# ur-whitelab/hoomd-tf

Hardware: AMD Instinct MI355X
Metric: MD steps/sec + achieved HBM GB/s, 131072 particles NN=128 (131k-particle box of the BASELINE metric) (higher is better)
Workload: dtype f32

## Files before the change

### hoomd_tf_amd/csrc/standin.hip

```cpp
#include <cstdlib>

#include "htf_common.h"
#include "box_math.h"
#include "htf_standin.h"
#include "standin_gate.h"
#include "key_sort.h"

namespace htf {

template <typename T>
__global__ __launch_bounds__(256) void nve_step_kernel(typename Vec4<T>::type *__restrict__ pos,
                                                       typename Vec4<T>::type *__restrict__ vel,
                                                       const typename Vec4<T>::type *__restrict__ force,
                                                       unsigned N, T dt, SBox<T> b) {
    unsigned i = blockIdx.x * blockDim.x + threadIdx.x;
    if (i >= N) return;
    auto p = pos[i];
    auto v = vel[i];
    nve_advance<T>(p, v, force[i], dt, b);
    pos[i] = p;
    vel[i] = v;
}

template <typename T>
__global__ __launch_bounds__(1024) void max_disp_kernel(const typename Vec4<T>::type *__restrict__ pos,
                                                        const typename Vec4<T>::type *__restrict__ ref, unsigned N,
                                                        SBox<T> b, float *__restrict__ out) {
    __shared__ float s_max[16];
    unsigned i = blockIdx.x * blockDim.x + threadIdx.x;
    float d2 = 0.f;
    if (i < N) {
        auto p = pos[i];
        auto r = ref[i];
        T dx = mimg<T>(p.x - r.x, b.L[0], b.Linv[0], b.periodic[0]);
        T dy = mimg<T>(p.y - r.y, b.L[1], b.Linv[1], b.periodic[1]);
        T dz = mimg<T>(p.z - r.z, b.L[2], b.Linv[2], b.periodic[2]);
        d2 = (float)(dx * dx + dy * dy + dz * dz);
        if (!(d2 == d2)) d2 = 0.f;
    }
    for (int m = 1; m < 64; m <<= 1) d2 = fmaxf(d2, __shfl_xor(d2, m));
    if ((threadIdx.x & 63) == 0) s_max[threadIdx.x >> 6] = d2;
    __syncthreads();
    if (threadIdx.x < 16) {
        d2 = s_max[threadIdx.x];
        for (int m = 1; m < 16; m <<= 1) d2 = fmaxf(d2, __shfl_xor(d2, m));
        if (threadIdx.x == 0 && __float_as_uint(d2) > *(volatile unsigned *)out)
            atomicMax((unsigned *)out, __float_as_uint(d2));
    }
}

template <typename T>
__global__ __launch_bounds__(1024) void check_disp_kernel(const typename Vec4<T>::type *__restrict__ pos,
                                                          const typename Vec4<T>::type *__restrict__ ref, unsigned N,
                                                          SBox<T> b, unsigned *__restrict__ work, float *__restrict__ out,
                                                          float *__restrict__ h_out, htfs_mirror mirror) {
    __shared__ float s_max[16];
    __shared__ unsigned s_last;
    unsigned i = blockIdx.x * blockDim.x + threadIdx.x;
    float d2 = 0.f;
    if (i < N) {
        auto p = pos[i];
        auto r = ref[i];
        T dx = mimg<T>(p.x - r.x, b.L[0], b.Linv[0], b.periodic[0]);
        T dy = mimg<T>(p.y - r.y, b.L[1], b.Linv[1], b.periodic[1]);
        T dz = mimg<T>(p.z - r.z, b.L[2], b.Linv[2], b.periodic[2]);
        d2 = (float)(dx * dx + dy * dy + dz * dz);
        if (!(d2 == d2)) d2 = 0.f;
    }
    for (int m = 1; m < 64; m <<= 1) d2 = fmaxf(d2, __shfl_xor(d2, m));
    if ((threadIdx.x & 63) == 0) s_max[threadIdx.x >> 6] = d2;
    if (threadIdx.x == 0) s_last = 0u;
    __syncthreads();
    if (threadIdx.x < 16) {
        d2 = s_max[threadIdx.x];
        for (int m = 1; m < 16; m <<= 1) d2 = fmaxf(d2, __shfl_xor(d2, m));
        if (threadIdx.x == 0) {
            if (__float_as_uint(d2) > *(volatile unsigned *)work) atomicMax(work, __float_as_uint(d2));
            __threadfence();
            if (atomicAdd(work + 1, 1u) == gridDim.x - 1u) s_last = 1u;
        }
    }
    __syncthreads();
    if (s_last == 0u) return;
    for (unsigned m = 0; m < mirror.n; ++m) {
        const unsigned *src = (const unsigned *)mirror.src[m];
        unsigned *dst = (unsigned *)mirror.dst[m];
        for (unsigned w = threadIdx.x; w < mirror.words[m]; w += blockDim.x) dst[w] = __builtin_nontemporal_load(src + w);
    }
    __threadfence_system();
    __syncthreads();
    if (threadIdx.x == 0) {
        const float worst = __uint_as_float(atomicExch(work, 0u));
        const unsigned cycle = __float_as_uint(out[1]) + 1u;
        out[0] = worst;
        out[1] = __uint_as_float(cycle);
        work[1] = 0u;
        if (h_out != nullptr) {
            h_out[0] = worst;
            __threadfence_system();
            *(volatile unsigned *)(h_out + 1) = cycle;
        }
    }
}

template <typename T>
__device__ __forceinline__ int cell_coord(T x, T lo, T Linv, int n) {
    int c = (int)floor((x - lo) * Linv * (T)n);
    return c < 0 ? 0 : (c >= n ? n - 1 : c);
}

template <typename T>
__global__ __launch_bounds__(256) void cell_index_kernel(const typename Vec4<T>::type *__restrict__ pos, unsigned Ntot,
                                                         SBox<T> b, int nx, int ny, int nz,
                                                         unsigned *__restrict__ cell_of, Gate gate) {
    if (gate.closed()) return;
    unsigned i = blockIdx.x * blockDim.x + threadIdx.x;
    if (i >= Ntot) return;
    auto p = pos[i];
    if (is_inert(p.x)) {
        cell_of[i] = kDeadCell;
        return;
    }
    int cx = cell_coord<T>(p.x, b.lo[0], b.Linv[0], nx);
    int cy = cell_coord<T>(p.y, b.lo[1], b.Linv[1], ny);
    int cz = cell_coord<T>(p.z, b.lo[2], b.Linv[2], nz);
    cell_of[i] = (unsigned)((cz * ny + cy) * nx + cx);
}

constexpr unsigned kTagSide = 1u << 31;
constexpr unsigned kRangeWrapShift = 28u, kRangeLenMask = (1u << kRangeWrapShift) - 1u;
struct RangesArgs {
    int nx, ny, nz, wx, wy, wz, px, py, pz;
    const unsigned *cell_start;
    uint4 *table;
    unsigned *max_neigh;
};
__device__ __forceinline__ void cell_ranges_body(const unsigned t, const RangesArgs &a) {
    const int nx = a.nx, ny = a.ny, nz = a.nz, wx = a.wx, wy = a.wy, wz = a.wz, px = a.px, py = a.py, pz = a.pz;
    const unsigned *__restrict__ cell_start = a.cell_start;
    uint4 *__restrict__ table = a.table;
    unsigned *__restrict__ max_neigh = a.max_neigh;
    const int nrow = (2 * wy + 1) * (2 * wz + 1);
    if (t == 0) *max_neigh = 0u;
    const unsigned ncell = (unsigned)(nx * ny * nz);
    if (t >= ncell * (unsigned)nrow) return;
    const int c = (int)(t / nrow), r = (int)(t % nrow);
    const int cx = c % nx, cy = (c / nx) % ny, cz = c / (nx * ny);
    const int dz = r / (2 * wy + 1) - wz, dy = r % (2 * wy + 1) - wy;
    int a0 = cx - wx, a1 = cx + wx, b0 = 0, b1 = -1;
    if (a0 < 0) {
        if (px) { b0 = nx + a0; b1 = nx - 1; }
        a0 = 0;
    } else if (a1 >= nx) {
// ... 234 lines not shown
            const unsigned i = my_tag & ~kTagSide;
            if (i < N) {
                n_neigh[i] = cnt < pitch ? cnt : pitch;
                head_list[i] = i * pitch;
                if (cnt > *(volatile unsigned *)max_neigh) atomicMax(max_neigh, cnt);
            }
        }
    }
}

}

using namespace htf;

extern "C" int htfs_nve_step(void *d_pos, void *d_vel, const void *d_force, int dtype, unsigned N, double dt,
                             const htf_box *box, htf_stream stream) {
    HTF_REQUIRE(d_pos && d_vel && d_force && box, "htfs_nve_step: null pointer");
    if (N == 0) return HTF_OK;
    unsigned grid = (N + 255) / 256;
    if (dtype == HTF_F32)
        hipLaunchKernelGGL((nve_step_kernel<float>), dim3(grid), dim3(256), 0, (hipStream_t)stream, (float4 *)d_pos, (float4 *)d_vel, (const float4 *)d_force, N, (float)dt, make_sbox<float>(box));
    else
        hipLaunchKernelGGL((nve_step_kernel<double>), dim3(grid), dim3(256), 0, (hipStream_t)stream, (double4 *)d_pos, (double4 *)d_vel, (const double4 *)d_force, N, dt, make_sbox<double>(box));
    return check_launch("nve_step_kernel");
}

extern "C" int htfs_max_displacement2(const void *d_pos, const void *d_ref, int dtype, unsigned N, const htf_box *box,
                                      float *d_out, htf_stream stream) {
    HTF_REQUIRE(d_pos && d_ref && box && d_out, "htfs_max_displacement2: null pointer");
    if (N == 0) return HTF_OK;
    unsigned grid = (N + 1023) / 1024;
    if (dtype == HTF_F32)
        hipLaunchKernelGGL((max_disp_kernel<float>), dim3(grid), dim3(1024), 0, (hipStream_t)stream, (const float4 *)d_pos, (const float4 *)d_ref, N, make_sbox<float>(box), d_out);
    else
        hipLaunchKernelGGL((max_disp_kernel<double>), dim3(grid), dim3(1024), 0, (hipStream_t)stream, (const double4 *)d_pos, (const double4 *)d_ref, N, make_sbox<double>(box), d_out);
    return check_launch("max_disp_kernel");
}

extern "C" int htfs_check_displacement2(const void *d_pos, const void *d_ref, int dtype, unsigned N, const htf_box *box,
                                        unsigned *d_work, float *d_out, float *h_out, const htfs_mirror *mirror, htf_stream stream) {
    using namespace htf;
    HTF_REQUIRE(d_pos && d_ref && box && d_work && d_out, "htfs_check_displacement2: null pointer");
    HTF_REQUIRE(N > 0, "htfs_check_displacement2: no rows");
    htfs_mirror mr = {};
    if (mirror != nullptr) {
        mr = *mirror;
        HTF_REQUIRE(mr.n <= HTFS_MIRROR_MAX, "htfs_check_displacement2: %u mirrors (at most %d)", mr.n, HTFS_MIRROR_MAX);
        for (unsigned m = 0; m < mr.n; ++m)
            HTF_REQUIRE(mr.src[m] && mr.dst[m] && ((uintptr_t)mr.src[m] & 3) == 0 && ((uintptr_t)mr.dst[m] & 3) == 0,
                        "htfs_check_displacement2: mirror %u: null or unaligned pointer", m);
    }
    unsigned grid = (N + 1023) / 1024;
    if (dtype == HTF_F32)
        hipLaunchKernelGGL((check_disp_kernel<float>), dim3(grid), dim3(1024), 0, (hipStream_t)stream, (const float4 *)d_pos, (const float4 *)d_ref, N, make_sbox<float>(box), d_work, d_out, h_out, mr);
    else
        hipLaunchKernelGGL((check_disp_kernel<double>), dim3(grid), dim3(1024), 0, (hipStream_t)stream, (const double4 *)d_pos, (const double4 *)d_ref, N, make_sbox<double>(box), d_work, d_out, h_out, mr);
    return check_launch("check_disp_kernel");
}

namespace htf {
struct Reimage {
    double L[3], c[3];
};
template <typename T>
__device__ __forceinline__ T reimage1(T x, double L, double c) {
    return L > 0.0 ? (T)((double)x - L * rint(((double)x - c) / L)) : x;
}

template <typename V>
__global__ __launch_bounds__(256) void bins_finish_kernel(RangesArgs ra, unsigned nb_ranges, V *__restrict__ dest, const V *__restrict__ src,
                                                          const int *__restrict__ order, unsigned n, int type_split, V *__restrict__ ref,
                                                          unsigned n_ref, unsigned *__restrict__ counter, Reimage im, Gate gate) {
    if (gate.closed()) return;
    if (blockIdx.x < nb_ranges) {
        cell_ranges_body(blockIdx.x * blockDim.x + threadIdx.x, ra);
        return;
    }
    const unsigned i = (blockIdx.x - nb_ranges) * blockDim.x + threadIdx.x;
    if (i == 0 && counter != nullptr) *counter += 1u;
    if (i >= n || i >= ra.cell_start[ra.nx * ra.ny * ra.nz]) return;
    const unsigned k = (unsigned)order[i];
    V p = src[k];
    if (ref != nullptr && k < n_ref) ref[k] = p;
    p.x = reimage1(p.x, im.L[0], im.c[0]);
    p.y = reimage1(p.y, im.L[1], im.c[1]);
    p.z = reimage1(p.z, im.L[2], im.c[2]);
    set_tag(p.w, k | ((type_split >= 0 && scalar_as_int(p.w) >= type_split) ? kTagSide : 0u));
    dest[i] = p;
}

template <typename T>
__global__ __launch_bounds__(256) void cell_index_count_kernel(const typename Vec4<T>::type *__restrict__ pos, unsigned Ntot, SBox<T> b,
                                                               int nx, int ny, int nz, unsigned *__restrict__ cell_of,
                                                               unsigned *__restrict__ count, Reimage im, Gate gate) {
    if (gate.closed()) return;
    unsigned i = blockIdx.x * blockDim.x + threadIdx.x;
    if (i >= Ntot) return;
    auto p = pos[i];
    if (is_inert(p.x)) {
        cell_of[i] = kDeadCell;
        return;
    }
    int cx = cell_coord<T>(reimage1(p.x, im.L[0], im.c[0]), b.lo[0], b.Linv[0], nx);
    int cy = cell_coord<T>(reimage1(p.y, im.L[1], im.c[1]), b.lo[1], b.Linv[1], ny);
    int cz = cell_coord<T>(reimage1(p.z, im.L[2], im.c[2]), b.lo[2], b.Linv[2], nz);
    const unsigned c = (unsigned)((cz * ny + cy) * nx + cx);
    cell_of[i] = c;
    atomicAdd(&count[c], 1u);
}

template <typename V, bool TAG>
__global__ void gather4_kernel(V *__restrict__ dest, const V *__restrict__ src, const int *__restrict__ order, unsigned n,
                               int type_split, Gate gate, const unsigned *__restrict__ n_live = nullptr) {
    if (gate.closed()) return;
    const unsigned i = blockIdx.x * blockDim.x + threadIdx.x;
    if (i >= n) return;
    if (n_live != nullptr && i >= *n_live) return;
    const unsigned k = (unsigned)order[i];
    V p = src[k];
    if (TAG) set_tag(p.w, k | ((type_split >= 0 && scalar_as_int(p.w) >= type_split) ? kTagSide : 0u));
    dest[i] = p;
}
}

namespace htf {
__global__ __launch_bounds__(256) void cell_count_kernel(const unsigned *__restrict__ cell_of, unsigned n,
                                                         unsigned *__restrict__ count, Gate gate) {
    if (gate.closed()) return;
    const unsigned i = blockIdx.x * blockDim.x + threadIdx.x;
    if (i < n && cell_of[i] != kDeadCell) atomicAdd(&count[cell_of[i]], 1u);
}

constexpr unsigned kScanThreads = 256, kScanPer = 8, kScanChunk = kScanThreads * kScanPer;
__global__ __launch_bounds__(kScanThreads) void cell_scan_kernel(const unsigned *__restrict__ count, unsigned ncell,
                                                         unsigned *__restrict__ start, unsigned *__restrict__ cursor, Gate gate) {
    if (gate.closed()) return;
    __shared__ unsigned s_wave[kScanThreads / 64], s_carry[kScanThreads / 64];
    const unsigned t = threadIdx.x, lane = t & 63u, wave = t >> 6;
    const unsigned base = blockIdx.x * kScanChunk;
    unsigned before_blk = 0;
    {
// ... 18 lines not shown
        const unsigned v = (unsigned)__shfl_up((int)incl, off);
        if (lane >= off) incl += v;
    }
    if (lane == 63) s_wave[wave] = incl;
    __syncthreads();
    unsigned before = 0, total = 0, carry = 0;
#pragma unroll
    for (unsigned w = 0; w < kScanThreads / 64; ++w) {
        const unsigned v = s_wave[w];
        before += w < wave ? v : 0u;
        total += v;
        carry += s_carry[w];
    }
    unsigned run = carry + before + (incl - sum);
#pragma unroll
    for (unsigned i = 0; i < kScanPer; ++i)
        if (first + i < ncell) {
            start[first + i] = run;
            cursor[first + i] = run;
            run += c[i];
        }
    if (blockIdx.x == gridDim.x - 1 && t == 0) start[ncell] = carry + total;
}

__global__ __launch_bounds__(256) void cell_scatter_kernel(const unsigned *__restrict__ cell_of, unsigned n,
                                                           unsigned *__restrict__ cursor, unsigned *__restrict__ order, Gate gate) {
    if (gate.closed()) return;
    const unsigned i = blockIdx.x * blockDim.x + threadIdx.x;
    if (i < n && cell_of[i] != kDeadCell) order[atomicAdd(&cursor[cell_of[i]], 1u)] = i;
}

__global__ __launch_bounds__(256) void cell_order_kernel(const unsigned *__restrict__ start, unsigned ncell,
                                                         unsigned *__restrict__ order, unsigned *__restrict__ count, Gate gate) {
    if (gate.closed()) return;
    const unsigned c = blockIdx.x * blockDim.x + threadIdx.x;
    if (c >= ncell) return;
    count[c] = 0u;
    const unsigned b = start[c], e = start[c + 1];
    for (unsigned i = b + 1; i < e; ++i) {
        const unsigned v = order[i];
        unsigned j = i;
        while (j > b && order[j - 1] > v) {
            order[j] = order[j - 1];
            --j;
        }
        order[j] = v;
    }
}
}

static int zero_counts(unsigned *count, unsigned ncell, hipStream_t s) {
    HTF_REQUIRE(((uintptr_t)count & 15) == 0, "binning scratch must be 16-byte aligned (cell_scan_kernel reads it with 16-byte loads)");
    HTF_CHECK_HIP(hipMemsetAsync(count, 0, (size_t)ncell * sizeof(unsigned), s));
    return HTF_OK;
}

extern "C" int htfs_cell_sort(const unsigned *d_cell_of, unsigned Ntot, unsigned ncell, unsigned *d_scratch,
                              unsigned *d_cell_start, unsigned *d_order, htf_stream stream) {
    using namespace htf;
    HTF_REQUIRE(d_cell_of && d_scratch && d_cell_start && d_order, "htfs_cell_sort: null pointer");
    HTF_REQUIRE(ncell > 0, "htfs_cell_sort: no cells");
    hipStream_t s = (hipStream_t)stream;
    unsigned *count = d_scratch, *cursor = d_scratch + ncell;
    if (int rc = zero_counts(count, ncell, s)) return rc;
    if (Ntot) hipLaunchKernelGGL(cell_count_kernel, dim3((Ntot + 255) / 256), dim3(256), 0, s, d_cell_of, Ntot, count, kOpenGate);
    hipLaunchKernelGGL(cell_scan_kernel, dim3((ncell + kScanChunk - 1) / kScanChunk), dim3(kScanThreads), 0, s, count, ncell, d_cell_start, cursor, kOpenGate);
    if (Ntot) hipLaunchKernelGGL(cell_scatter_kernel, dim3((Ntot + 255) / 256), dim3(256), 0, s, d_cell_of, Ntot, cursor, d_order, kOpenGate);
    hipLaunchKernelGGL(cell_order_kernel, dim3((ncell + 255) / 256), dim3(256), 0, s, d_cell_start, ncell, d_order, count, kOpenGate);
    return check_launch("htfs_cell_sort");
}

static int gather4(void *d_dest, const void *d_src, const int *d_order, int dtype, unsigned n, bool tag, int type_split,
                   htf_stream stream, const unsigned *d_n_live = nullptr) {
    using namespace htf;
    HTF_REQUIRE(d_dest && d_src && d_order, "htfs_gather4_tagged: null pointer");
    HTF_REQUIRE(!tag || n <= kTagSide, "htfs_gather4_tagged: %u particles do not fit the 31-bit tag", n);
    if (n == 0) return HTF_OK;
    const dim3 grid((n + 255) / 256), block(256);
    hipStream_t s = (hipStream_t)stream;
    if (dtype == HTF_F32) {
        if (tag) hipLaunchKernelGGL((gather4_kernel<float4, true>), grid, block, 0, s, (float4 *)d_dest, (const float4 *)d_src, d_order, n, type_split, kOpenGate, d_n_live);
        else hipLaunchKernelGGL((gather4_kernel<float4, false>), grid, block, 0, s, (float4 *)d_dest, (const float4 *)d_src, d_order, n, type_split, kOpenGate, d_n_live);
    } else {
        if (tag) hipLaunchKernelGGL((gather4_kernel<double4, true>), grid, block, 0, s, (double4 *)d_dest, (const double4 *)d_src, d_order, n, type_split, kOpenGate, d_n_live);
        else hipLaunchKernelGGL((gather4_kernel<double4, false>), grid, block, 0, s, (double4 *)d_dest, (const double4 *)d_src, d_order, n, type_split, kOpenGate, d_n_live);
    }
    return check_launch("gather4_kernel");
}

extern "C" int htfs_gather4_tagged(void *d_dest, const void *d_src, const int *d_order, int dtype, unsigned n, int type_split,
                                   htf_stream stream) {
    return gather4(d_dest, d_src, d_order, dtype, n, true, type_split, stream);
}

extern "C" int htfs_gather4_tagged_live(void *d_dest, const void *d_src, const int *d_order, int dtype, unsigned n_max,
                                        const unsigned *d_n_live, int type_split, htf_stream stream) {
    HTF_REQUIRE(d_n_live, "htfs_gather4_tagged_live: null pointer");
    return gather4(d_dest, d_src, d_order, dtype, n_max, true, type_split, stream, d_n_live);
}

template <typename T, typename V4>
__global__ __launch_bounds__(256) void slab_classify_kernel(const V4 *__restrict__ pos, unsigned N, const T *__restrict__ bounds,
                                                            int world, int rank, T r_ghost, unsigned *__restrict__ key) {
    const unsigned i = blockIdx.x * blockDim.x + threadIdx.x;
    if (i >= N) return;
    const T x = pos[i].x;
// ... 40 lines not shown
                                                           unsigned row_words, SegTable t, unsigned total_rows) {
    const unsigned w = blockIdx.x * blockDim.x + threadIdx.x;
    if (w >= total_rows * row_words) return;
    unsigned row = w / row_words;
    const unsigned col = w - row * row_words;
    unsigned seg = 0;
#pragma unroll 1
    while (seg + 1 < t.n && row >= t.cnt[seg]) {
        row -= t.cnt[seg];
        ++seg;
    }
    dst[(size_t)(t.dst[seg] + row) * row_words + col] = src[(size_t)(t.src[seg] + row) * row_words + col];
}

extern "C" int htfs_segment_copy(void *d_dst, const void *d_src, unsigned row_bytes, unsigned n_segments,
                                 const unsigned *src_start, const unsigned *dst_start, const unsigned *count, htf_stream stream) {
    HTF_REQUIRE(d_dst && d_src && src_start && dst_start && count, "htfs_segment_copy: null pointer");
    HTF_REQUIRE(n_segments >= 1 && n_segments <= HTFS_MAX_SEGMENTS && row_bytes % 4 == 0 && row_bytes > 0,
                "htfs_segment_copy: need 1..%d segments of whole 32-bit words", HTFS_MAX_SEGMENTS);
    SegTable t;
    t.n = 0;
    unsigned total = 0;
    for (unsigned s = 0; s < n_segments; ++s) {
        if (count[s] == 0) continue;
        t.src[t.n] = src_start[s];
        t.dst[t.n] = dst_start[s];
        t.cnt[t.n] = count[s];
        total += count[s];
        ++t.n;
    }
    if (total == 0) return HTF_OK;
    const unsigned words = row_bytes / 4;
    const unsigned grid = (unsigned)(((size_t)total * words + 255) / 256);
    hipLaunchKernelGGL(segment_copy_kernel, dim3(grid), dim3(256), 0, (hipStream_t)stream, (unsigned *)d_dst, (const unsigned *)d_src,
                       words, t, total);
    return check_launch("segment_copy_kernel");
}

extern "C" int htfs_cell_index(const void *d_pos, int dtype, unsigned Ntot, const htf_box *box, const int *ncell3,
                               unsigned *d_cell_of, htf_stream stream) {
    HTF_REQUIRE(d_pos && box && ncell3 && d_cell_of, "htfs_cell_index: null pointer");
    if (Ntot == 0) return HTF_OK;
    unsigned grid = (Ntot + 255) / 256;
    if (dtype == HTF_F32)
        hipLaunchKernelGGL((cell_index_kernel<float>), dim3(grid), dim3(256), 0, (hipStream_t)stream, (const float4 *)d_pos, Ntot, make_sbox<float>(box), ncell3[0], ncell3[1], ncell3[2], d_cell_of, kOpenGate);
    else
        hipLaunchKernelGGL((cell_index_kernel<double>), dim3(grid), dim3(256), 0, (hipStream_t)stream, (const double4 *)d_pos, Ntot, make_sbox<double>(box), ncell3[0], ncell3[1], ncell3[2], d_cell_of, kOpenGate);
    return check_launch("cell_index_kernel");
}

struct FinishArgs {
    unsigned n;
    htf::Reimage im;
};

static int build_nlist_impl(const htfs_nlist *l, const void *d_pos, int dtype, unsigned N, htf_stream stream, htf::Gate gate,
                            const FinishArgs *fin) {
    using namespace htf;
    HTF_REQUIRE(l && d_pos && l->pos_sorted && l->cell_start && l->n_neigh && l->head_list && l->nlist && l->max_neigh,
                "htfs_build_nlist: null pointer");
    const htf_box *box = &l->box;
    const int *ncell3 = l->ncell3, *stencil3 = l->stencil3;
    const unsigned *d_cell_start = l->cell_start;
    const void *d_pos_sorted = l->pos_sorted;
    const unsigned pitch = l->pitch;
    const int type_split = l->type_split;
    const double r_list = l->r_list;
    unsigned *d_n_neigh = l->n_neigh, *d_head_list = l->head_list, *d_nlist = l->nlist, *d_max_neigh = l->max_neigh;
    HTF_REQUIRE(pitch > 0, "htfs_build_nlist: pitch must be > 0");
    for (int d = 0; d < 3; ++d) {
        const double w = (box->hi[d] - box->lo[d]) / ncell3[d];
        const int sw = stencil3[d];
        HTF_REQUIRE((sw == 0 && ncell3[d] == 1) || (sw >= 1 && sw <= 2 && ncell3[d] >= 2 * sw + 1 && w * sw >= r_list * (1.0 - 1e-12)),
                    "htfs_build_nlist: along %d need 1 cell, or >= 2w+1 cells with w cells spanning r_list (got %d cells of %g, stencil %d, r_list %g)",
                    d, ncell3[d], w, sw, r_list);
    }
    if (N == 0) return HTF_OK;
    const unsigned ncell = (unsigned)(ncell3[0] * ncell3[1] * ncell3[2]);
    const unsigned nrow = (unsigned)((2 * stencil3[1] + 1) * (2 * stencil3[2] + 1));
    HTF_REQUIRE(l->ranges && ((uintptr_t)l->ranges & 15) == 0, "htfs_build_nlist: ranges must be a 16-byte aligned table of 4 * ncell * rows words");
    uint4 *d_ranges = (uint4 *)l->ranges;
    const RangesArgs ra = {ncell3[0], ncell3[1], ncell3[2], stencil3[0], stencil3[1], stencil3[2], (int)box->periodic[0],
                           (int)box->periodic[1], (int)box->periodic[2], d_cell_start, d_ranges, d_max_neigh};
    const unsigned nb_ranges = (ncell * nrow + 255) / 256;
    if (fin == nullptr) {
        hipLaunchKernelGGL(cell_ranges_kernel, dim3(nb_ranges), dim3(256), 0, (hipStream_t)stream, ra, gate);
    } else {
        const unsigned nb = nb_ranges + (fin->n + 255) / 256 + (fin->n == 0 ? 1u : 0u);
        if (dtype == HTF_F32)
            hipLaunchKernelGGL((bins_finish_kernel<float4>), dim3(nb), dim3(256), 0, (hipStream_t)stream, ra, nb_ranges, (float4 *)l->pos_sorted,
                               (const float4 *)d_pos, (const int *)l->order, fin->n, type_split, (float4 *)l->ref, N, l->counter, fin->im, gate);
        else
            hipLaunchKernelGGL((bins_finish_kernel<double4>), dim3(nb), dim3(256), 0, (hipStream_t)stream, ra, nb_ranges, (double4 *)l->pos_sorted,
                               (const double4 *)d_pos, (const int *)l->order, fin->n, type_split, (double4 *)l->ref, N, l->counter, fin->im, gate);
    }
    const bool fine = stencil3[0] == 2 || stencil3[1] == 2 || stencil3[2] == 2;
#define HTFS_NL(T, V4, G)                                                                                              \
    if (shift) HTFS_NL_(T, V4, G, true); else HTFS_NL_(T, V4, G, false)
#define HTFS_NL_(T, V4, G, S)                                                                                          \
    hipLaunchKernelGGL((build_nlist_kernel<T, G, S>), dim3((N + 4 * (64 / G) - 1) / (4 * (64 / G))), dim3(256), 0, (hipStream_t)stream, \
                       (const V4 *)d_pos, (const V4 *)d_pos_sorted, N, make_sbox<T>(box), (T)(r_list * r_list), ncell3[0],  \
                       ncell3[1], ncell3[2], stencil3[0], stencil3[1], stencil3[2], d_cell_start, pitch,      \
                       type_split, d_n_neigh, d_head_list, d_nlist, d_max_neigh, (const uint4 *)d_ranges, gate)
#define HTFS_NLC(T, V4)                                                                                                \
    if (shift) HTFS_NLC_(T, V4, true); else HTFS_NLC_(T, V4, false)
#define HTFS_NLC_(T, V4, S)                                                                                            \
    hipLaunchKernelGGL((build_nlist_cells_kernel<T, S>), dim3((ncell * cell_split + 3) / 4), dim3(256), 0, (hipStream_t)stream, \
                       (const V4 *)d_pos_sorted, N, make_sbox<T>(box), (T)(r_list * r_list), ncell, (int)nrow, d_cell_start, pitch, \
                       type_split, d_n_neigh, d_head_list, d_nlist, d_max_neigh, (const uint4 *)d_ranges, cell_split, gate)
    bool shift = true;
    for (int d = 0; d < 3; ++d) shift = shift && (!box->periodic[d] || ncell3[d] >= 7);
#ifdef HTF_AB_VARIANTS
    static const bool per_particle = std::getenv("HTFS_NLIST_PER_PARTICLE") != nullptr, per_cell = std::getenv("HTFS_NLIST_PER_CELL") != nullptr;
#else
    constexpr bool per_particle = false, per_cell = false;
#endif
    const bool reimaged = fin != nullptr && (fin->im.L[0] > 0.0 || fin->im.L[1] > 0.0 || fin->im.L[2] > 0.0);
    const bool by_cell = per_cell || reimaged || (!per_particle && ncell >= 1024u);
    const unsigned cell_split = ncell <= 12288u ? 2u : 1u;
    if (by_cell) {
        if (dtype == HTF_F32) { HTFS_NLC(float, float4); } else { HTFS_NLC(double, double4); }
    } else if (dtype == HTF_F32) {
        if (fine) { HTFS_NL(float, float4, 8); } else { HTFS_NL(float, float4, 16); }
    } else {
        if (fine) { HTFS_NL(double, double4, 8); } else { HTFS_NL(double, double4, 16); }
    }
#undef HTFS_NL
#undef HTFS_NL_
#undef HTFS_NLC
#undef HTFS_NLC_
    return check_launch("build_nlist_kernel");
}

extern "C" int htfs_build_nlist(const htfs_nlist *nl, const void *d_pos, int dtype, unsigned N, htf_stream stream) {
    return build_nlist_impl(nl, d_pos, dtype, N, stream, htf::kOpenGate, nullptr);
}

static int rebuild_nlist_impl(const htfs_nlist *l, const void *d_pos, int dtype, unsigned N, unsigned Ntot, bool scratch_clean,
                              htf_stream stream, htf::Gate gate) {
    using namespace htf;
    HTF_REQUIRE(l && d_pos && l->cell_of && l->scratch && l->cell_start && l->order && l->pos_sorted, "htfs_rebuild_nlist: null pointer");
    HTF_REQUIRE(Ntot >= N, "htfs_rebuild_nlist: Ntot %u < N %u", Ntot, N);
    if (N == 0) return HTF_OK;
    const htf_box *box = &l->box;
    const int *ncell3 = l->ncell3;
    const unsigned ncell = (unsigned)(ncell3[0] * ncell3[1] * ncell3[2]);
    HTF_REQUIRE(ncell > 0, "htfs_rebuild_nlist: no cells");
    hipStream_t s = (hipStream_t)stream;
    unsigned *count = l->scratch, *cursor = l->scratch + ncell;
    if (!scratch_clean)
        if (int rc = zero_counts(count, ncell, s)) return rc;
    const unsigned grid = (Ntot + 255) / 256;
    Reimage im = {};
    for (int d = 0; d < 3; ++d) {
        im.L[d] = !box->periodic[d] ? l->image_L[d] : 0.0;
        im.c[d] = 0.5 * (box->lo[d] + box->hi[d]);
        HTF_REQUIRE(im.L[d] == 0.0 || im.L[d] >= box->hi[d] - box->lo[d], "htfs_rebuild_nlist: image length %g along axis %d is shorter than the grid", im.L[d], d);
    }
    if (dtype == HTF_F32)
        hipLaunchKernelGGL((cell_index_count_kernel<float>), dim3(grid), dim3(256), 0, s, (const float4 *)d_pos, Ntot, make_sbox<float>(box),
                           ncell3[0], ncell3[1], ncell3[2], l->cell_of, count, im, gate);
    else
        hipLaunchKernelGGL((cell_index_count_kernel<double>), dim3(grid), dim3(256), 0, s, (const double4 *)d_pos, Ntot, make_sbox<double>(box),
                           ncell3[0], ncell3[1], ncell3[2], l->cell_of, count, im, gate);
    hipLaunchKernelGGL(cell_scan_kernel, dim3((ncell + kScanChunk - 1) / kScanChunk), dim3(kScanThreads), 0, s, count, ncell, l->cell_start, cursor, gate);
    hipLaunchKernelGGL(cell_scatter_kernel, dim3(grid), dim3(256), 0, s, l->cell_of, Ntot, cursor, l->order, gate);
    hipLaunchKernelGGL(cell_order_kernel, dim3((ncell + 255) / 256), dim3(256), 0, s, l->cell_start, ncell, l->order, count, gate);
    const FinishArgs fin = {Ntot, im};
    return build_nlist_impl(l, d_pos, dtype, N, stream, gate, &fin);
}

extern "C" int htfs_rebuild_nlist(const htfs_nlist *nl, const void *d_pos, int dtype, unsigned N, unsigned Ntot, int scratch_clean,
                                  htf_stream stream) {
    return rebuild_nlist_impl(nl, d_pos, dtype, N, Ntot, scratch_clean != 0, stream, htf::kOpenGate);
}

extern "C" int htfs_check_rebuild_nlist(const htfs_nlist *nl, const void *d_pos, int dtype, unsigned N, unsigned Ntot, int scratch_clean,
                                        float *d_disp2, double threshold2, unsigned *d_stat2, unsigned *h_stat2, htf_stream stream) {
    HTF_REQUIRE(nl && nl->ref && d_disp2 && d_stat2, "htfs_check_rebuild_nlist: null pointer");
    if (N == 0) return HTF_OK;
    HTF_CHECK_HIP(hipMemsetAsync(d_disp2, 0, sizeof(float), (hipStream_t)stream));
    int rc = htfs_max_displacement2(d_pos, nl->ref, dtype, N, &nl->box, d_disp2, stream);
    if (rc != HTF_OK) return rc;
    htfs_nlist l = *nl;
    l.max_neigh = d_stat2;
    l.counter = d_stat2 + 1;
    rc = rebuild_nlist_impl(&l, d_pos, dtype, N, Ntot, scratch_clean != 0, stream, htf::Gate{d_disp2, (float)threshold2});
    if (rc != HTF_OK) return rc;
    if (h_stat2 != nullptr)
        HTF_CHECK_HIP(hipMemcpyAsync(h_stat2, d_stat2, 2 * sizeof(unsigned), hipMemcpyDeviceToHost, (hipStream_t)stream));
    return HTF_OK;
}
```

### hoomd_tf_amd/standin.py

```python
import ctypes as C
import math
import os

import numpy as np
import torch

from . import _lib, ops
from ._lib import lib, check
from .ops import raw_stream


def fcc_positions(n_cells, rho):
    a = (4.0 / rho) ** (1.0 / 3.0)
    L = n_cells * a
    ijk = np.stack(np.meshgrid(*[np.arange(n_cells)] * 3, indexing="ij"), -1).reshape(-1, 3)
    base = np.array([[0.25, 0.25, 0.25], [0.75, 0.75, 0.25], [0.75, 0.25, 0.75], [0.25, 0.75, 0.75]])
    pos = ((ijk[:, None, :] + base[None]) * a).reshape(-1, 3) - L / 2
    return pos, np.array([L, L, L]), a


def sc_positions(n_cells, rho):
    a = (1.0 / rho) ** (1.0 / 3.0)
    L = n_cells * a
    ijk = np.stack(np.meshgrid(*[np.arange(n_cells)] * 3, indexing="ij"), -1).reshape(-1, 3)
# ... 123 lines not shown
        self._capturing = False
        self._stat = self._stat_host = self._stat_event = None
        self._max_host = self._max_event = None
        self._mirrored = False

    def subscribe(self, rcut_fn):
        self._subscribers.append(rcut_fn)
        self.r_cut = max([self.r_cut] + [float(fn()) for fn in self._subscribers])
        self._ref = None

    @property
    def r_list(self):
        return self.r_cut + self.r_buff

    def _ncell(self):
        b3, _ = self._search_box()
        L = b3[1] - b3[0]
        n = np.ones(3, dtype=int)
        w = np.zeros(3, dtype=int)
        for d in range(3):
            fine = int(np.floor(L[d] / (self.r_list / 2.0)))
            coarse = int(np.floor(L[d] / self.r_list))
            if fine >= 5:
                n[d], w[d] = fine, 2
            elif coarse >= 3:
                n[d], w[d] = coarse, 1
        return n, w

    def _search_box(self):
        if self.domain is not None and getattr(self.domain, "local_grid", False):
            return self.domain.nlist_box()
        return self.sys.box3x3, self.sys.periodic

    def _size_grid(self):
        s, d = self.sys, self._desc
        b3, per = self._search_box()
        key = (np.asarray(b3).tobytes(), per)
        if self._sbox_key != key:
            self._sbox_key = key
            d.box = _lib.make_box(np.asarray(b3), per)
        n, w = self._ncell()
        ncell = int(n[0] * n[1] * n[2])
        Ntot = s.N + s.n_ghost
        d.r_list = self.r_list
        d.ncell3[:] = [int(x) for x in n]
        d.stencil3[:] = [int(x) for x in w]
        lengths = getattr(self.domain, "image_lengths", None)
        d.image_L[:] = lengths() if lengths is not None else (0.0, 0.0, 0.0)
        if self._scr_n != (Ntot, ncell, int(w[1]), int(w[2])):
            self._scr_n = (Ntot, ncell, int(w[1]), int(w[2]))
            self._cell_of = torch.empty(Ntot, dtype=torch.int32, device=s.device)
            self._order = torch.empty(Ntot, dtype=torch.int32, device=s.device)
            self._cell_start = torch.empty(ncell + 1, dtype=torch.int32, device=s.device)
            self._bin_scratch = torch.empty(2 * ncell, dtype=torch.int32, device=s.device)
            self._pos_sorted = torch.empty((Ntot, 4), dtype=s.pos.dtype, device=s.device)
            self._ranges = torch.empty(4 * ncell * int((2 * w[1] + 1) * (2 * w[2] + 1)), dtype=torch.int32, device=s.device)
            d.cell_of, d.order, d.cell_start = self._cell_of.data_ptr(), self._order.data_ptr(), self._cell_start.data_ptr()
            d.scratch, d.pos_sorted, d.ranges = self._bin_scratch.data_ptr(), self._pos_sorted.data_ptr(), self._ranges.data_ptr()
        self._grid = (n, w, ncell)
        return Ntot

    def build(self):
        s = self.sys
        if self.domain is not None:
            self.domain.rebuild()
        Ntot = self._size_grid()
        fixed = self.domain is not None and getattr(self.domain, "fixed_capacity", False)
        if (fixed and self.n_builds > 0 and not self.sort_particles and self._ref is not None and self._ref.shape[0] == s.N
                and self.nlist is not None and self.nlist.numel() == s.N * self.pitch):
            self._rebuild_fixed(Ntot)
        else:
            self._build_sized(Ntot, fixed)
        if self._rule is not None:
            self._rule.reset()
            self._dd_prev = None
        self.n_builds += 1

    def _rebuild_fixed(self, Ntot):
        self._poll_max()
        self._enqueue_rebuild(Ntot, gated=False)
        self._copy_max_late()

    def _build_sized(self, Ntot, fixed):
        s, d = self.sys, self._desc
        n, _, ncell = self._grid
        cell_of = self._cell_of
        stream = C.c_void_p(raw_stream(s.device.index))
        check(lib.htfs_cell_index(s.pos.data_ptr(), s.scalar_code, Ntot, C.byref(d.box), C.byref(d.ncell3), d.cell_of, stream))
        if self.sort_particles and s.N > 0:
            key = cell_of[: s.N].to(torch.int64)
            if self.domain is not None and self.domain.world > 1:
                key = key + self.domain.row_classes() * ncell
            perm = torch.sort(key, stable=True)[1]
            s.pos[: s.N] = s.pos[: s.N].index_select(0, perm)
            s.vel = s.vel.index_select(0, perm)
            cell_of[: s.N] = cell_of[: s.N].index_select(0, perm)
        self._scratch_clean = None
        check(lib.htfs_cell_sort(d.cell_of, Ntot, ncell, d.scratch, d.cell_start, d.order, stream))
        self._scratch_clean = (d.scratch, ncell)
        if fixed:
            check(lib.htfs_gather4_tagged_live(d.pos_sorted, s.pos.data_ptr(), d.order, s.scalar_code, Ntot,
                                               d.cell_start + 4 * ncell, int(self.type_split), stream))
        else:
            check(lib.htfs_gather4_tagged(d.pos_sorted, s.pos.data_ptr(), d.order, s.scalar_code, Ntot, int(self.type_split), stream))
        if self.pitch is None:
            L = s.box3x3[1] - s.box3x3[0]
            n_real = getattr(self.domain, "n_global", None) if fixed else None
# ... 656 lines not shown
```

### include/htf_standin.h

```cpp
#ifndef HTF_STANDIN_H_
#define HTF_STANDIN_H_
#include "htf_amd.h"
#ifdef __cplusplus
extern "C" {
#endif

HTF_API int htfs_nve_step(void *d_pos, void *d_vel, const void *d_force, int dtype, unsigned N,
                          double dt, const htf_box *box, htf_stream stream);

HTF_API int htfs_max_displacement2(const void *d_pos, const void *d_ref, int dtype, unsigned N,
                                   const htf_box *box, float *d_out, htf_stream stream);

#define HTFS_MIRROR_MAX 4
typedef struct htfs_mirror {
    const void *src[HTFS_MIRROR_MAX];
    void *dst[HTFS_MIRROR_MAX];
    unsigned words[HTFS_MIRROR_MAX];
    unsigned n;
} htfs_mirror;
HTF_API int htfs_check_displacement2(const void *d_pos, const void *d_ref, int dtype, unsigned N, const htf_box *box,
                                     unsigned *d_work, float *d_out, float *h_out, const htfs_mirror *mirror, htf_stream stream);

#define HTFS_RANGE_WORDS(ncell, stencil_y, stencil_z) (4u * (size_t)(ncell) * (2u * (stencil_y) + 1u) * (2u * (stencil_z) + 1u))
typedef struct htfs_nlist {
    htf_box box;
    double r_list;
    int ncell3[3];
    int stencil3[3];
    unsigned pitch;
    int type_split;
    unsigned *cell_of;
    unsigned *scratch;
    unsigned *cell_start;
    unsigned *order;
    void *pos_sorted;
    void *ranges;
    unsigned *n_neigh;
    unsigned *head_list;
    unsigned *nlist;
    unsigned *max_neigh;
    void *ref;
    unsigned *counter;
    double image_L[3];
} htfs_nlist;

HTF_API int htfs_cell_index(const void *d_pos, int dtype, unsigned Ntot, const htf_box *box,
                            const int *ncell3, unsigned *d_cell_of, htf_stream stream);
HTF_API int htfs_cell_sort(const unsigned *d_cell_of, unsigned Ntot, unsigned ncell, unsigned *d_scratch,
                           unsigned *d_cell_start, unsigned *d_order, htf_stream stream);
HTF_API int htfs_gather4_tagged(void *d_dest, const void *d_src, const int *d_order, int dtype, unsigned n, int type_split,
                                htf_stream stream);
HTF_API int htfs_gather4_tagged_live(void *d_dest, const void *d_src, const int *d_order, int dtype, unsigned n_max,
                                     const unsigned *d_n_live, int type_split, htf_stream stream);
HTF_API int htfs_build_nlist(const htfs_nlist *nl, const void *d_pos, int dtype, unsigned N, htf_stream stream);

HTF_API int htfs_rebuild_nlist(const htfs_nlist *nl, const void *d_pos, int dtype, unsigned N, unsigned Ntot, int scratch_clean,
                               htf_stream stream);

HTF_API int htfs_check_rebuild_nlist(const htfs_nlist *nl, const void *d_pos, int dtype, unsigned N, unsigned Ntot, int scratch_clean,
                                     float *d_disp2, double threshold2, unsigned *d_stat2, unsigned *h_stat2, htf_stream stream);

HTF_API int htfs_slab_classify(const void *d_pos, int dtype, unsigned N, const void *d_bounds, int world, int rank,
                               double r_ghost, unsigned *d_key, htf_stream stream);

HTF_API int htfs_key_sort16(const unsigned *d_key, unsigned N, unsigned *d_scratch, unsigned *d_start, unsigned *d_order,
                            htf_stream stream);

#define HTFS_MAX_SEGMENTS 16
HTF_API int htfs_segment_copy(void *d_dst, const void *d_src, unsigned row_bytes, unsigned n_segments,
                              const unsigned *src_start, const unsigned *dst_start, const unsigned *count, htf_stream stream);

#define HTFS_BRICK_MAX_MSG 8
#define HTFS_BRICK_MAX_P 64
typedef struct htfs_brick {
    int ndim;
    int axis[2];
// ... 123 lines not shown
```

Measured before the change: 13280.

## Fold cell ordering into bins_finish and fuse displacement check with counter reset

Removes the separate cell_order_kernel. The scatter now writes into a staging buffer, and bins_finish computes each particle's deterministic in-cell slot by counting smaller indices within its cell, while also zeroing the cell counts. The nlist rebuild check replaces a memset plus max_disp launch with a single check_disp_kernel variant that resets its work counters itself, so later memsets are skipped. The cost is an O(cell occupancy) scan per particle and a larger scratch buffer.

```diff
diff --git a/hoomd_tf_amd/csrc/standin.hip b/hoomd_tf_amd/csrc/standin.hip
--- a/hoomd_tf_amd/csrc/standin.hip
+++ b/hoomd_tf_amd/csrc/standin.hip
@@ -23,10 +23,9 @@
 }
 
 template <typename T>
-__global__ __launch_bounds__(1024) void max_disp_kernel(const typename Vec4<T>::type *__restrict__ pos,
-                                                        const typename Vec4<T>::type *__restrict__ ref, unsigned N,
-                                                        SBox<T> b, float *__restrict__ out) {
-    __shared__ float s_max[16];
+__device__ __forceinline__ float block_max_disp2(const typename Vec4<T>::type *__restrict__ pos,
+                                                 const typename Vec4<T>::type *__restrict__ ref, unsigned N, const SBox<T> &b,
+                                                 float *s_max) {
     unsigned i = blockIdx.x * blockDim.x + threadIdx.x;
     float d2 = 0.f;
     if (i < N) {
@@ -44,61 +43,57 @@
     if (threadIdx.x < 16) {
         d2 = s_max[threadIdx.x];
         for (int m = 1; m < 16; m <<= 1) d2 = fmaxf(d2, __shfl_xor(d2, m));
-        if (threadIdx.x == 0 && __float_as_uint(d2) > *(volatile unsigned *)out)
-            atomicMax((unsigned *)out, __float_as_uint(d2));
-    }
+    }
+    return d2;
 }
 
 template <typename T>
+__global__ __launch_bounds__(1024) void max_disp_kernel(const typename Vec4<T>::type *__restrict__ pos,
+                                                        const typename Vec4<T>::type *__restrict__ ref, unsigned N,
+                                                        SBox<T> b, float *__restrict__ out) {
+    __shared__ float s_max[16];
+    const float d2 = block_max_disp2<T>(pos, ref, N, b, s_max);
+    if (threadIdx.x == 0 && __float_as_uint(d2) > *(volatile unsigned *)out)
+        atomicMax((unsigned *)out, __float_as_uint(d2));
+}
+
+template <typename T, bool CYCLE>
 __global__ __launch_bounds__(1024) void check_disp_kernel(const typename Vec4<T>::type *__restrict__ pos,
                                                           const typename Vec4<T>::type *__restrict__ ref, unsigned N,
                                                           SBox<T> b, unsigned *__restrict__ work, float *__restrict__ out,
                                                           float *__restrict__ h_out, htfs_mirror mirror) {
     __shared__ float s_max[16];
     __shared__ unsigned s_last;
-    unsigned i = blockIdx.x * blockDim.x + threadIdx.x;
-    float d2 = 0.f;
-    if (i < N) {
-        auto p = pos[i];
-        auto r = ref[i];
-        T dx = mimg<T>(p.x - r.x, b.L[0], b.Linv[0], b.periodic[0]);
-        T dy = mimg<T>(p.y - r.y, b.L[1], b.Linv[1], b.periodic[1]);
-        T dz = mimg<T>(p.z - r.z, b.L[2], b.Linv[2], b.periodic[2]);
-        d2 = (float)(dx * dx + dy * dy + dz * dz);
-        if (!(d2 == d2)) d2 = 0.f;
-    }
-    for (int m = 1; m < 64; m <<= 1) d2 = fmaxf(d2, __shfl_xor(d2, m));
-    if ((threadIdx.x & 63) == 0) s_max[threadIdx.x >> 6] = d2;
     if (threadIdx.x == 0) s_last = 0u;
-    __syncthreads();
-    if (threadIdx.x < 16) {
-        d2 = s_max[threadIdx.x];
-        for (int m = 1; m < 16; m <<= 1) d2 = fmaxf(d2, __shfl_xor(d2, m));
-        if (threadIdx.x == 0) {
-            if (__float_as_uint(d2) > *(volatile unsigned *)work) atomicMax(work, __float_as_uint(d2));
-            __threadfence();
-            if (atomicAdd(work + 1, 1u) == gridDim.x - 1u) s_last = 1u;
-        }
+    const float d2 = block_max_disp2<T>(pos, ref, N, b, s_max);
+    if (threadIdx.x == 0) {
+        if (__float_as_uint(d2) > *(volatile unsigned *)work) atomicMax(work, __float_as_uint(d2));
+        __threadfence();
+        if (atomicAdd(work + 1, 1u) == gridDim.x - 1u) s_last = 1u;
     }
     __syncthreads();
     if (s_last == 0u) return;
-    for (unsigned m = 0; m < mirror.n; ++m) {
-        const unsigned *src = (const unsigned *)mirror.src[m];
-        unsigned *dst = (unsigned *)mirror.dst[m];
-        for (unsigned w = threadIdx.x; w < mirror.words[m]; w += blockDim.x) dst[w] = __builtin_nontemporal_load(src + w);
-    }
-    __threadfence_system();
-    __syncthreads();
+    if (CYCLE) {
+        for (unsigned m = 0; m < mirror.n; ++m) {
+            const unsigned *src = (const unsigned *)mirror.src[m];
+            unsigned *dst = (unsigned *)mirror.dst[m];
+            for (unsigned w = threadIdx.x; w < mirror.words[m]; w += blockDim.x) dst[w] = __builtin_nontemporal_load(src + w);
+        }
+        __threadfence_system();
+        __syncthreads();
+    }
     if (threadIdx.x == 0) {
         const float worst = __uint_as_float(atomicExch(work, 0u));
-        const unsigned cycle = __float_as_uint(out[1]) + 1u;
         out[0] = worst;
-        out[1] = __uint_as_float(cycle);
         work[1] = 0u;
-        if (h_out != nullptr) {
-            h_out[0] = worst;
-            __threadfence_system();
-            *(volatile unsigned *)(h_out + 1) = cycle;
+        if (CYCLE) {
+            const unsigned cycle = __float_as_uint(out[1]) + 1u;
+            out[1] = __uint_as_float(cycle);
+            if (h_out != nullptr) {
+                h_out[0] = worst;
+                __threadfence_system();
+                *(volatile unsigned *)(h_out + 1) = cycle;
+            }
         }
     }
 }
@@ -439,9 +434,9 @@
     }
     unsigned grid = (N + 1023) / 1024;
     if (dtype == HTF_F32)
-        hipLaunchKernelGGL((check_disp_kernel<float>), dim3(grid), dim3(1024), 0, (hipStream_t)stream, (const float4 *)d_pos, (const float4 *)d_ref, N, make_sbox<float>(box), d_work, d_out, h_out, mr);
+        hipLaunchKernelGGL((check_disp_kernel<float, true>), dim3(grid), dim3(1024), 0, (hipStream_t)stream, (const float4 *)d_pos, (const float4 *)d_ref, N, make_sbox<float>(box), d_work, d_out, h_out, mr);
     else
-        hipLaunchKernelGGL((check_disp_kernel<double>), dim3(grid), dim3(1024), 0, (hipStream_t)stream, (const double4 *)d_pos, (const double4 *)d_ref, N, make_sbox<double>(box), d_work, d_out, h_out, mr);
+        hipLaunchKernelGGL((check_disp_kernel<double, true>), dim3(grid), dim3(1024), 0, (hipStream_t)stream, (const double4 *)d_pos, (const double4 *)d_ref, N, make_sbox<double>(box), d_work, d_out, h_out, mr);
     return check_launch("check_disp_kernel");
 }
 
@@ -456,24 +451,33 @@
 
 template <typename V>
 __global__ __launch_bounds__(256) void bins_finish_kernel(RangesArgs ra, unsigned nb_ranges, V *__restrict__ dest, const V *__restrict__ src,
-                                                          const int *__restrict__ order, unsigned n, int type_split, V *__restrict__ ref,
-                                                          unsigned n_ref, unsigned *__restrict__ counter, Reimage im, Gate gate) {
+                                                          const unsigned *__restrict__ stage, const unsigned *__restrict__ cell_of,
+                                                          unsigned *__restrict__ order, unsigned *__restrict__ count, unsigned n,
+                                                          int type_split, V *__restrict__ ref, unsigned n_ref,
+                                                          unsigned *__restrict__ counter, Reimage im, Gate gate) {
     if (gate.closed()) return;
     if (blockIdx.x < nb_ranges) {
-        cell_ranges_body(blockIdx.x * blockDim.x + threadIdx.x, ra);
+        const unsigned t = blockIdx.x * blockDim.x + threadIdx.x;
+        if (count != nullptr && t < (unsigned)(ra.nx * ra.ny * ra.nz)) count[t] = 0u;
+        cell_ranges_body(t, ra);
         return;
     }
     const unsigned i = (blockIdx.x - nb_ranges) * blockDim.x + threadIdx.x;
     if (i == 0 && counter != nullptr) *counter += 1u;
     if (i >= n || i >= ra.cell_start[ra.nx * ra.ny * ra.nz]) return;
-    const unsigned k = (unsigned)order[i];
+    const unsigned k = stage[i];
     V p = src[k];
+    const unsigned c = cell_of[k];
+    const unsigned cb = ra.cell_start[c], ce = ra.cell_start[c + 1];
+    unsigned slot = cb;
+    for (unsigned j = cb; j < ce; ++j) slot += stage[j] < k ? 1u : 0u;
+    order[slot] = k;
     if (ref != nullptr && k < n_ref) ref[k] = p;
     p.x = reimage1(p.x, im.L[0], im.c[0]);
     p.y = reimage1(p.y, im.L[1], im.c[1]);
     p.z = reimage1(p.z, im.L[2], im.c[2]);
     set_tag(p.w, k | ((type_split >= 0 && scalar_as_int(p.w) >= type_split) ? kTagSide : 0u));
-    dest[i] = p;
+    dest[slot] = p;
 }
 
 template <typename T>
@@ -598,6 +602,13 @@
 static int zero_counts(unsigned *count, unsigned ncell, hipStream_t s) {
     HTF_REQUIRE(((uintptr_t)count & 15) == 0, "binning scratch must be 16-byte aligned (cell_scan_kernel reads it with 16-byte loads)");
     HTF_CHECK_HIP(hipMemsetAsync(count, 0, (size_t)ncell * sizeof(unsigned), s));
+    return HTF_OK;
+}
+static int zero_nlist_scratch(const htfs_nlist *l, hipStream_t s) {
+    const unsigned ncell = (unsigned)(l->ncell3[0] * l->ncell3[1] * l->ncell3[2]);
+    HTF_REQUIRE(l->scratch && ncell > 0, "htfs_rebuild_nlist: no scratch, or no cells");
+    if (int rc = zero_counts(l->scratch, ncell, s)) return rc;
+    HTF_CHECK_HIP(hipMemsetAsync(l->scratch + HTFS_SCRATCH_WORK(ncell), 0, 2 * sizeof(unsigned), s));
     return HTF_OK;
 }
 
@@ -744,6 +755,8 @@
 struct FinishArgs {
     unsigned n;
     htf::Reimage im;
+    const unsigned *stage;
+    unsigned *count;
 };
 
 static int build_nlist_impl(const htfs_nlist *l, const void *d_pos, int dtype, unsigned N, htf_stream stream, htf::Gate gate,
@@ -781,10 +794,10 @@
         const unsigned nb = nb_ranges + (fin->n + 255) / 256 + (fin->n == 0 ? 1u : 0u);
         if (dtype == HTF_F32)
             hipLaunchKernelGGL((bins_finish_kernel<float4>), dim3(nb), dim3(256), 0, (hipStream_t)stream, ra, nb_ranges, (float4 *)l->pos_sorted,
-                               (const float4 *)d_pos, (const int *)l->order, fin->n, type_split, (float4 *)l->ref, N, l->counter, fin->im, gate);
+                               (const float4 *)d_pos, fin->stage, l->cell_of, l->order, fin->count, fin->n, type_split, (float4 *)l->ref, N, l->counter, fin->im, gate);
         else
             hipLaunchKernelGGL((bins_finish_kernel<double4>), dim3(nb), dim3(256), 0, (hipStream_t)stream, ra, nb_ranges, (double4 *)l->pos_sorted,
-                               (const double4 *)d_pos, (const int *)l->order, fin->n, type_split, (double4 *)l->ref, N, l->counter, fin->im, gate);
+                               (const double4 *)d_pos, fin->stage, l->cell_of, l->order, fin->count, fin->n, type_split, (double4 *)l->ref, N, l->counter, fin->im, gate);
     }
     const bool fine = stencil3[0] == 2 || stencil3[1] == 2 || stencil3[2] == 2;
 #define HTFS_NL(T, V4, G)                                                                                              \
@@ -839,9 +852,9 @@
     const unsigned ncell = (unsigned)(ncell3[0] * ncell3[1] * ncell3[2]);
     HTF_REQUIRE(ncell > 0, "htfs_rebuild_nlist: no cells");
     hipStream_t s = (hipStream_t)stream;
-    unsigned *count = l->scratch, *cursor = l->scratch + ncell;
+    unsigned *count = l->scratch, *cursor = l->scratch + ncell, *stage = l->scratch + HTFS_SCRATCH_STAGE(ncell);
     if (!scratch_clean)
-        if (int rc = zero_counts(count, ncell, s)) return rc;
+        if (int rc = zero_nlist_scratch(l, s)) return rc;
     const unsigned grid = (Ntot + 255) / 256;
     Reimage im = {};
     for (int d = 0; d < 3; ++d) {
@@ -856,9 +869,8 @@
         hipLaunchKernelGGL((cell_index_count_kernel<double>), dim3(grid), dim3(256), 0, s, (const double4 *)d_pos, Ntot, make_sbox<double>(box),
                            ncell3[0], ncell3[1], ncell3[2], l->cell_of, count, im, gate);
     hipLaunchKernelGGL(cell_scan_kernel, dim3((ncell + kScanChunk - 1) / kScanChunk), dim3(kScanThreads), 0, s, count, ncell, l->cell_start, cursor, gate);
-    hipLaunchKernelGGL(cell_scatter_kernel, dim3(grid), dim3(256), 0, s, l->cell_of, Ntot, cursor, l->order, gate);
-    hipLaunchKernelGGL(cell_order_kernel, dim3((ncell + 255) / 256), dim3(256), 0, s, l->cell_start, ncell, l->order, count, gate);
-    const FinishArgs fin = {Ntot, im};
+    hipLaunchKernelGGL(cell_scatter_kernel, dim3(grid), dim3(256), 0, s, l->cell_of, Ntot, cursor, stage, gate);
+    const FinishArgs fin = {Ntot, im, stage, count};
     return build_nlist_impl(l, d_pos, dtype, N, stream, gate, &fin);
 }
 
@@ -869,17 +881,29 @@
 
 extern "C" int htfs_check_rebuild_nlist(const htfs_nlist *nl, const void *d_pos, int dtype, unsigned N, unsigned Ntot, int scratch_clean,
                                         float *d_disp2, double threshold2, unsigned *d_stat2, unsigned *h_stat2, htf_stream stream) {
-    HTF_REQUIRE(nl && nl->ref && d_disp2 && d_stat2, "htfs_check_rebuild_nlist: null pointer");
+    using namespace htf;
+    HTF_REQUIRE(nl && nl->ref && nl->scratch && d_pos && d_disp2 && d_stat2, "htfs_check_rebuild_nlist: null pointer");
     if (N == 0) return HTF_OK;
-    HTF_CHECK_HIP(hipMemsetAsync(d_disp2, 0, sizeof(float), (hipStream_t)stream));
-    int rc = htfs_max_displacement2(d_pos, nl->ref, dtype, N, &nl->box, d_disp2, stream);
+    const unsigned ncell = (unsigned)(nl->ncell3[0] * nl->ncell3[1] * nl->ncell3[2]);
+    HTF_REQUIRE(ncell > 0, "htfs_check_rebuild_nlist: no cells");
+    hipStream_t s = (hipStream_t)stream;
+    unsigned *work = nl->scratch + HTFS_SCRATCH_WORK(ncell);
+    if (!scratch_clean)
+        if (int rc = zero_nlist_scratch(nl, s)) return rc;
+    const unsigned grid = (N + 1023) / 1024;
+    const htfs_mirror none = {};
+    if (dtype == HTF_F32)
+        hipLaunchKernelGGL((check_disp_kernel<float, false>), dim3(grid), dim3(1024), 0, s, (const float4 *)d_pos, (const float4 *)nl->ref, N, make_sbox<float>(&nl->box), work, d_disp2, (float *)nullptr, none);
+    else
+        hipLaunchKernelGGL((check_disp_kernel<double, false>), dim3(grid), dim3(1024), 0, s, (const double4 *)d_pos, (const double4 *)nl->ref, N, make_sbox<double>(&nl->box), work, d_disp2, (float *)nullptr, none);
+    int rc = check_launch("check_disp_kernel");
     if (rc != HTF_OK) return rc;
     htfs_nlist l = *nl;
     l.max_neigh = d_stat2;
     l.counter = d_stat2 + 1;
-    rc = rebuild_nlist_impl(&l, d_pos, dtype, N, Ntot, scratch_clean != 0, stream, htf::Gate{d_disp2, (float)threshold2});
+    rc = rebuild_nlist_impl(&l, d_pos, dtype, N, Ntot, true, stream, Gate{d_disp2, (float)threshold2});
     if (rc != HTF_OK) return rc;
     if (h_stat2 != nullptr)
-        HTF_CHECK_HIP(hipMemcpyAsync(h_stat2, d_stat2, 2 * sizeof(unsigned), hipMemcpyDeviceToHost, (hipStream_t)stream));
+        HTF_CHECK_HIP(hipMemcpyAsync(h_stat2, d_stat2, 2 * sizeof(unsigned), hipMemcpyDeviceToHost, s));
     return HTF_OK;
 }
diff --git a/hoomd_tf_amd/standin.py b/hoomd_tf_amd/standin.py
--- a/hoomd_tf_amd/standin.py
+++ b/hoomd_tf_amd/standin.py
@@ -199,7 +199,7 @@
             self._cell_of = torch.empty(Ntot, dtype=torch.int32, device=s.device)
             self._order = torch.empty(Ntot, dtype=torch.int32, device=s.device)
             self._cell_start = torch.empty(ncell + 1, dtype=torch.int32, device=s.device)
-            self._bin_scratch = torch.empty(2 * ncell, dtype=torch.int32, device=s.device)
+            self._bin_scratch = torch.zeros(2 * ncell + 2 + Ntot, dtype=torch.int32, device=s.device)
             self._pos_sorted = torch.empty((Ntot, 4), dtype=s.pos.dtype, device=s.device)
             self._ranges = torch.empty(4 * ncell * int((2 * w[1] + 1) * (2 * w[2] + 1)), dtype=torch.int32, device=s.device)
             d.cell_of, d.order, d.cell_start = self._cell_of.data_ptr(), self._order.data_ptr(), self._cell_start.data_ptr()
diff --git a/include/htf_standin.h b/include/htf_standin.h
--- a/include/htf_standin.h
+++ b/include/htf_standin.h
@@ -22,6 +22,9 @@
                                      unsigned *d_work, float *d_out, float *h_out, const htfs_mirror *mirror, htf_stream stream);
 
 #define HTFS_RANGE_WORDS(ncell, stencil_y, stencil_z) (4u * (size_t)(ncell) * (2u * (stencil_y) + 1u) * (2u * (stencil_z) + 1u))
+#define HTFS_SCRATCH_WORK(ncell) (2u * (size_t)(ncell))
+#define HTFS_SCRATCH_STAGE(ncell) (HTFS_SCRATCH_WORK(ncell) + 2u)
+#define HTFS_SCRATCH_WORDS(ncell, Ntot) (HTFS_SCRATCH_STAGE(ncell) + (size_t)(Ntot))
 typedef struct htfs_nlist {
     htf_box box;
     double r_list;
```

New measurement: 13460, median of 6. 1.01x the previous value.
